# nmndeep/Robust-Segmentation

Hardware: AMD Instinct MI355X
Metric: SEA attack-iterations/sec (UperNet-CNX-T, 512x512) (higher is better)
Workload: dtype f32 (frozen-weight GEMMs on the 16-bit matrix cores by operand splitting: fp16x2 (22 significant bits per operand, 3 MFMA products) forward, fp16x2 (22 significant bits per operand, 3 MFMA products) input gradient; fp32 storage and accumulate)

## Files before the change

include/sea_hip.h:

```cpp
#ifndef SEA_HIP_H
#define SEA_HIP_H

#include <stddef.h>
#include <stdint.h>

#ifdef __cplusplus
extern "C" {
#endif

#define SEA_MODE_MASK_CE 0
#define SEA_MODE_MASK_CE_BAL 1
#define SEA_MODE_JS 2
#define SEA_MODE_CE 3

#define SEA_DTYPE_F32 0
#define SEA_DTYPE_BF16 1
#define SEA_DTYPE_F16 2

#define SEA_LAYOUT_NCHW 0
#define SEA_LAYOUT_NHWC 1

int sea_abi_version(void);
const char* sea_build_info(void);
#define SEA_CONFIG_XCD_ORDER 0
// ... 147 lines not shown
int sea_nhwc_to_nchw(const float* in, const float* scale, const float* residual, float* out, int B, int C,
                     int64_t HW, void* stream);

int sea_patch2x2(const float* src, float* dst, int B, int H, int W, int C, int inverse, void* stream);

int sea_attention_bwd_terms(const float* q, const float* k, const float* v, int64_t sb, int64_t sh, int64_t st, int B, int H,
                            int T, int D, float scale, const float* out, const float* grad_out, const float* lse,
                            float* delta, float* dq, float* dk, float* dv, int64_t gsb, int64_t gsh, int64_t gst,
                            int terms, void* stream);
int sea_attention_fwd_terms(const float* q, const float* k, const float* v, int64_t sb, int64_t sh, int64_t st, int B, int H,
                            int T, int D, float scale, float* out, float* lse, int terms, void* stream);
int sea_attention_fwd_f16(const float* q, const float* k, const float* v, int64_t sb, int64_t sh, int64_t st, int B, int H,
                          int T, int D, float scale, uint32_t* amax_ws, float* out, float* lse, void* stream);
int sea_attention_bwd_f16(const float* q, const float* k, const float* v, int64_t sb, int64_t sh, int64_t st, int B, int H,
                          int T, int D, float scale, const float* out, const float* grad_out, const float* lse,
                          float* delta, uint32_t* amax_ws, float* dq, float* dk, float* dv, int64_t gsb, int64_t gsh,
                          int64_t gst, void* stream);

#define SEA_GEMM_VARIANT_DEFAULT 0u
#define SEA_GEMM_PIPE_SINGLE 1u
#define SEA_GEMM_PIPE_PINGPONG 2u
#define SEA_GEMM_PIPE_BIG 3u
#define SEA_GEMM_PIPE_MASK 3u
#define SEA_GEMM_SHAPE16 4u
int sea_gemm_plan(int M, int N, int K, int terms, int batch, int64_t lda, int64_t ldc, int64_t ld_addend, int prologue, int fused,
                  unsigned variant, int32_t out[16]);
int64_t sea_gemm_split_packed_bytes(int N, int K, int terms);
int sea_absmax_bits(const float* A, int64_t lda, int M, int K, int batch, int64_t strideA, int rows_per_word,
                    uint32_t* out_bits, void* stream);
int sea_gemm_split_f16(const float* A, int64_t lda, const void* Wp, float* C, int64_t ldc, const float* bias, int relu, int M,
                       int N, int K, int batch, int64_t strideA, int64_t strideW_bytes, int64_t strideC,
                       const uint32_t* amax_bits, int amax_rows, uint32_t* out_amax, unsigned variant, void* stream);
int sea_gemm_split_pack(const float* W, int64_t ldw, int trans, int N, int K, int terms, void* out, void* stream);
int sea_gemm_splitk_reduce(const float* partial, int splits, int M, int N, const float* bias, const float* addend,
                           int64_t ld_addend, int relu, float* C, int64_t ldc, uint32_t* out_amax, void* stream);
typedef struct SeaGemmEpilogue {
  const float* addend;
  int64_t ld_addend, stride_addend;
  float* gelu_out;
  const float* gelu_grad_of;
  const float* a_gelu_grad_of;
  int a_gate;
  int a_gelu;
  float a_amax_mul;
  const float* a_amax_mul_dev;
} SeaGemmEpilogue;
int sea_gemm_split_fused(const float* A, int64_t lda, const void* Wp, float* C, int64_t ldc, const float* bias, int relu, int M,
                         int N, int K, int terms, int batch, int64_t strideA, int64_t strideW_bytes, int64_t strideC,
                         const uint32_t* amax_bits, int amax_rows, uint32_t* out_amax, const SeaGemmEpilogue* epi,
                         unsigned variant, void* stream);
int sea_gemm_split(const float* A, int64_t lda, const void* Wp, float* C, int64_t ldc, const float* bias, int relu, int M,
                   int N, int K, int terms, int batch, int64_t strideA, int64_t strideW_bytes, int64_t strideC,
                   unsigned variant, void* stream);
int sea_classifier_supported(int P, int K, int cls);
int sea_classifier_fwd(const float* y, const float* W, const float* bias, float* out, int B, int P, int K, int cls, void* stream);
int sea_classifier_bwd(const float* g, const float* W, float* gy, int B, int P, int K, int cls, const float* gate,
                       const float* gate_scale, void* stream);
int sea_mlp_fused_supported(int C, int H);
int sea_ln_mlp_fused_fwd(const float* x, int64_t ldx, const float* ln_w, const float* ln_b, float ln_eps, const void* W1p,
                         const float* b1, const void* W2p, const float* b2, const float* res, int64_t ldres, float* y,
                         int64_t ldy, int M, int C, int H, const uint32_t* amax_x, const uint32_t* amax_h, void* stream);
int sea_ln_mlp_fused_bwd(const float* g, int64_t ldg, const float* x, int64_t ldx, const float* ln_w, const float* ln_b,
                         float ln_eps, const void* W1p, const float* b1, const void* W2tp, const void* W1tp, float* dx,
                         int64_t lddx, int M, int C, int H, const uint32_t* amax_x, const float* amax_mul_dev, void* stream);
int sea_probe_gelu_mismatches(unsigned long long* out, void* stream);
int sea_probe_ln_rows(const float* x, const float* ln_w, const float* ln_b, float eps, int M, int C, float* yn, float* mean,
                      float* rstd, void* stream);
int sea_mlp_fused_stamps(int bwd, const float* g, int64_t ldg, const float* x, int64_t ldx, const void* W1p, const float* b1,
                         const void* W2p, const void* W1tp, const float* b2, const float* res, float* y, int M, int C,
                         const uint32_t* amax_x, const uint32_t* amax_h, const float* amax_mul_dev, unsigned long long* dbg,
                         void* stream);
int sea_mlp_fused_fwd(const float* x, int64_t ldx, const void* W1p, const float* b1, const void* W2p, const float* b2,
                      const float* res, int64_t ldres, float* y, int64_t ldy, int M, int C, int H, const uint32_t* amax_x,
                      const uint32_t* amax_h, void* stream);
int sea_mlp_fused_bwd(const float* g, int64_t ldg, const float* x, int64_t ldx, const void* W1p, const float* b1,
                      const void* W2tp, const void* W1tp, float* dx, int64_t lddx, int M, int C, int H,
                      const uint32_t* amax_x, const float* amax_mul_dev, void* stream);
int sea_probe_stream_copy(const void* src, void* dst, size_t bytes, int non_temporal, void* stream);
int sea_probe_stream_read(const void* src, float* sink, size_t bytes, void* stream);

#define SEA_MSF_MAX_CLASSES 192
int sea_msf_resize_input(const float* x, float* y, float* y_flip, int64_t planes, int h, int w, int H, int W,
                         void* stream);
int sea_msf_accumulate(const float* logits, float* score, int B, int C, int hl, int wl, int Hs, int Ws, int H, int W,
                       int flip, void* stream);

#define SEA_SW_MAX_ANCHORS 32
int sea_sw_merge(const float* logits, float* out, int B, int C, int hl, int wl, int ws, const int* h_anchors, int n_h,
                 const int* w_anchors, int n_w, int H, int W, int flip, int softmax, int accumulate, void* stream);
int sea_sw_finish(const float* avg, float* score, int B, int C, int H, int W, int Ho, int Wo, int flip, int accumulate,
                  void* stream);

int sea_sw_cut(const float* x, float* crops, int B, int Cx, int ws, const int* h_anchors, int n_h, const int* w_anchors,
               int n_w, int H, int W, void* stream);
int sea_sw_cut_bwd(const float* dcrops, float* dx, int B, int Cx, int ws, const int* h_anchors, int n_h,
                   const int* w_anchors, int n_w, int H, int W, void* stream);
int sea_sw_merge_bwd(const float* g, float* dlogits, int B, int C, int hl, int wl, int ws, const int* h_anchors, int n_h,
                     const int* w_anchors, int n_w, int H, int W, void* stream);

int sea_psp_polyphase_split(const float* x, float* y, int B, int H, int W, int C, int d, int first_only, void* stream);
int sea_psp_polyphase_merge(const float* y, float* x, int B, int H, int W, int C, int d, int first_only, void* stream);
int sea_psp_upsample_ac(const float* x, float* y, int64_t planes, int h, int w, int H, int W, void* stream);
int sea_psp_upsample_ac_bwd(const float* gy, float* gx, float* work, int64_t planes, int h, int w, int H, int W,
                            void* stream);
int sea_psp_upsample_ac_nhwc(const float* x, float* y, int B, int C, int h, int w, int H, int W, int S, void* stream);
int sea_psp_upsample_ac_nhwc_bwd(const float* gy, float* gx, float* work, int B, int C, int h, int w, int H, int W,
// ... 56 lines not shown
```

robust-segmentation_amd/build_native.py:

```python
#!/usr/bin/env python3
from __future__ import annotations

import hashlib
import os
import shutil
import subprocess
import sys
from concurrent.futures import ThreadPoolExecutor

HERE = os.path.dirname(os.path.abspath(__file__))
CSRC = os.path.join(HERE, "csrc")
LIBDIR = os.path.join(HERE, "lib")
OBJDIR = os.path.join(HERE, "build")
LIB = os.path.join(LIBDIR, "libsea_hip.so")
ARCH = "gfx950"

SOURCES = [
    ("linf_kernels.hip", ["-ffp-contract=off"]),
    ("l2_kernels.hip", ["-ffp-contract=off"]),
    ("apgd_control.hip", ["-ffp-contract=off"]),
    ("loss_kernels.hip", []),
    ("loss_stream.hip", []),
    ("loss_split.hip", []),
    ("loss_upsampled.hip", []),
    ("stats_kernels.hip", []),
    ("dwconv_kernels.hip", []),
    ("upsample_kernels.hip", []),
    ("transpose_kernels.hip", ["-ffp-contract=off"]),
    ("wino_kernels.hip", []),
    ("ln_kernels.hip", []),
    ("block_tail.hip", ["-ffp-contract=off"]),
    ("stem_kernels.hip", []),
    ("fpn_fused.hip", []),
    ("probe_kernels.hip", []),
    ("attention.hip", []),
    ("attention_bf16.hip", []),
    ("gemm_split.hip", []),
    ("gemm_split_big.hip", ["-fno-slp-vectorize"]),
    ("gemm_split_pp.hip", ["-fno-slp-vectorize"]),
    ("mlp_fused.hip", ["-fno-slp-vectorize"]),
    ("classifier.hip", []),
    ("msf_kernels.hip", ["-ffp-contract=off"]),
    ("msf_grad.hip", ["-ffp-contract=off"]),
    ("sw_kernels.hip", ["-ffp-contract=off"]),
    ("psp_kernels.hip", []),
    ("bn_train.hip", []),
    ("train_loss.hip", []),
    ("train_loss_up.hip", []),
    ("train_loss_up_pow2.hip", []),
    ("greedy_host.cpp", ["-ffp-contract=off"]),
    ("api_misc.cpp", []),
]
HEADERS = ["sea_common.h", "attention_common.h", "colsum.h", "loss_common.h", "loss_plan.h", "gemm_plan.h", "upsample_plan.h", "launch_grid.h", "gemm_split.h", "bilinear_map.h", "msf_map.h", "train_loss_common.h", os.path.join("..", "..", "include", "sea_hip.h")]


def _hipcc() -> str:
    for cand in (os.environ.get("HIPCC"), shutil.which("hipcc"), "/opt/rocm/bin/hipcc"):
        if cand and os.path.exists(cand):
            return cand
    raise RuntimeError("hipcc not found (set HIPCC)")


def _digest() -> str:
    h = hashlib.sha256()
    for name, flags in SOURCES:
        h.update(open(os.path.join(CSRC, name), "rb").read())
        h.update(" ".join(flags).encode())
    for name in HEADERS:
        h.update(open(os.path.join(CSRC, name), "rb").read())
    return h.hexdigest()[:16]


def build(force: bool = False, verbose: bool = True) -> str:
    stamp_file = os.path.join(LIBDIR, "libsea_hip.stamp")
    digest = _digest()
    if not force and os.path.exists(LIB) and os.path.exists(stamp_file) and open(stamp_file).read() == digest:
        return LIB
    os.makedirs(LIBDIR, exist_ok=True)
    os.makedirs(OBJDIR, exist_ok=True)
    hipcc = _hipcc()
    common = ["-O3", "-fPIC", "-std=c++17", f"--offload-arch={ARCH}", "-Wno-unused-result"]

    hdr = hashlib.sha256()
    for name in HEADERS:
        hdr.update(open(os.path.join(CSRC, name), "rb").read())

    def compile_one(item):
        name, flags = item
        if name == "api_misc.cpp":
            flags = flags + [f'-DSEA_BUILD_STAMP="{digest}"']
        obj = os.path.join(OBJDIR, os.path.splitext(name)[0] + ".o")
        h = hdr.copy()
        h.update(open(os.path.join(CSRC, name), "rb").read())
        h.update(" ".join(common + flags).encode())
        key, keyfile = h.hexdigest(), obj + ".key"
        if not force and os.path.exists(obj) and os.path.exists(keyfile) and open(keyfile).read() == key:
            return obj
        cmd = [hipcc, *common, *flags, "-c", os.path.join(CSRC, name), "-o", obj]
        if verbose:
            print("[build]", " ".join(cmd), flush=True)
        subprocess.run(cmd, check=True)
        with open(keyfile, "w") as f:
            f.write(key)
        return obj

    with ThreadPoolExecutor(max_workers=min(4, len(SOURCES))) as ex:
# ... 15 lines not shown
```

robust-segmentation_amd/semseg/_native.py:

```python
from __future__ import annotations

import ctypes as C
import os
from typing import Optional

import torch

_PKG = os.path.dirname(os.path.dirname(os.path.abspath(__file__)))
LIB_PATH = os.environ.get("SEA_HIP_LIB", os.path.join(_PKG, "lib", "libsea_hip.so"))

MODE_BY_NAME = {"mask-ce-avg": 0, "mask-ce-bal": 1, "js-avg": 2, "ce": 3, "ce-avg": 3}
DTYPE_CODE = {torch.float32: 0, torch.bfloat16: 1, torch.float16: 2}
LAYOUT_NCHW, LAYOUT_NHWC = 0, 1

_lib = None

_vp, _i, _i64, _f, _sz, _u = C.c_void_p, C.c_int, C.c_int64, C.c_float, C.c_size_t, C.c_uint
_SIGS = {
    "sea_abi_version": (C.c_int, []),
    "sea_build_info": (C.c_char_p, []),
    "sea_fastdiv_magic": (_i, [C.c_uint32, C.POINTER(C.c_uint32), C.POINTER(C.c_uint32)]),
    "sea_apgd_linf_step": (_i, [_vp, _vp, _vp, _vp, _vp, _f, _f, _vp, _i, _i64, _vp]),
    "sea_apgd_l2_workspace_bytes": (_i64, [_i]),
    "sea_apgd_l2_step": (_i, [_vp, _vp, _vp, _vp, _vp, _f, _f, _vp, _vp, _i, _i64, _vp]),
# ... 17 lines not shown
    "sea_apgd_track_graph": (_i, [_vp, _vp, _vp, _vp, _i, _i64, _vp, _vp, _vp, _i, _vp, _vp, _vp, _vp, _vp, _vp, _vp, _vp,
                                  _vp, _vp, _vp]),
    "sea_select_copy": (_i, [_vp, _vp, _vp, _vp, _vp, _vp, _vp, _vp, _i, _i, _i64, _i64, _vp]),
    "sea_count_ignored": (_i, [_vp, _i, _i, _i64, _vp, _vp]),
    "sea_worst_miou_greedy": (_i, [_vp, _vp, _i, _i, _i, _vp, _i, _vp, _vp, _vp]),
    "sea_dwconv7x7": (_i, [_vp, _vp, _vp, _vp, _i, _i, _i, _i, _i, _vp]),
    "sea_dwconv7x7_nhwc": (_i, [_vp, _vp, _vp, _vp, _i, _i, _i, _i, _i, _u, _vp]),
    "sea_dwconv7x7_nhwc_add": (_i, [_vp, _vp, _vp, _vp, _vp, _i, _i, _i, _i, _i, _u, _vp]),
    "sea_nchw_to_nhwc": (_i, [_vp, _vp, _vp, _i, _i, _i64, _vp]),
    "sea_nhwc_to_nchw": (_i, [_vp, _vp, _vp, _vp, _i, _i, _i64, _vp]),
    "sea_upsample_bilinear_fwd": (_i, [_vp, _vp, _i64, _i, _i, _i, _i, _vp]),
    "sea_upsample_bilinear_bwd": (_i, [_vp, _vp, _i64, _i, _i, _i, _i, _vp]),
    "sea_layernorm_fwd": (_i, [_vp, _vp, _vp, _vp, _vp, _vp, _i64, _i, _f, _vp]),
    "sea_layernorm_bwd": (_i, [_vp, _vp, _vp, _vp, _vp, _vp, _i64, _i, _vp]),
    "sea_layernorm_bwd_params_workspace": (_i64, [_i64, _i]),
    "sea_layernorm_bwd_params": (_i, [_vp, _vp, _vp, _vp, _vp, _vp, _vp, _vp, _vp, _i64, _i, _vp]),
    "sea_block_tail_fwd": (_i, [_vp, _vp, _vp, _vp, _vp, _i64, _i, _i, _vp]),
    "sea_block_tail_bwd_workspace": (_i64, [_i64, _i]),
    "sea_block_tail_bwd": (_i, [_vp, _vp, _vp, _vp, _vp, _vp, _vp, _i64, _i, _i, _vp]),
    "sea_dwconv7x7_nhwc_wgrad_workspace": (_i64, [_i, _i, _i]),
    "sea_dwconv7x7_nhwc_wgrad": (_i, [_vp, _vp, _vp, _vp, _vp, _i, _i, _i, _i, _vp]),
    "sea_adaptive_avg_pool_nhwc_fwd": (_i, [_vp, _vp, _i, _i, _i, _i, _i, _i, _vp]),
    "sea_adaptive_avg_pool_nhwc_bwd": (_i, [_vp, _vp, _i, _i, _i, _i, _i, _i, _vp]),
    "sea_stem_conv1_ln_gelu": (_i, [_vp, _vp, _vp, _vp, _vp, _vp, _vp, _i, _i, _i, _i, _f, _vp]),
    "sea_stem_conv1_bwd": (_i, [_vp, _vp, _vp, _i, _i, _i, _i, _vp]),
    "sea_ln_gelu_cl_fwd": (_i, [_vp, _vp, _vp, _vp, _i, _i, _i, _i64, _f, _vp]),
    "sea_ln_gelu_cl_bwd": (_i, [_vp, _i, _vp, _vp, _vp, _vp, _i, _i, _i64, _f, _vp]),
    "sea_wino_tiles": (_i64, [_i, _i, _i, _i]),
    "sea_wino_input_transform": (_i, [_vp, _i64, _vp, _vp, _vp, _i64, _i, _i, _i, _i, _i, _i, _vp]),
    "sea_wino_filter_transform": (_i, [_vp, _vp, _i, _i, _i, _i, _vp]),
    "sea_wino_output_transform": (_i, [_vp, _vp, _vp, _vp, _i, _vp, _i, _i, _i, _i, _i, _i, _vp]),
    "sea_tap_gather_fwd": (_i, [_vp, _vp, _i, _i, _i, _i, _i, _i, _i, _i, _vp]),
    "sea_tap_gather_bwd": (_i, [_vp, _vp, _i, _i, _i, _i, _i, _i, _vp]),
    "sea_gate_scale": (_i, [_vp, _vp, _vp, _vp, _i64, _i, _vp]),
    "sea_upsample_bilinear_nhwc_fwd": (_i, [_vp, _vp, _vp, _i, _i, _i, _i, _i, _i, _i64, _vp]),
    "sea_upsample_bilinear_nhwc_bwd": (_i, [_vp, _vp, _i, _i, _i, _i, _i, _i, _i64, _vp]),
    "sea_upsample_plan": (_i, [_i, _i64, _i, _i, _i, _i, _i, _i64, _sz, _sz, _i, _i, C.POINTER(C.c_int32)]),
    "sea_patch2x2": (_i, [_vp, _vp, _i, _i, _i, _i, _i, _vp]),
    "sea_attention_bwd_terms": (_i, [_vp, _vp, _vp, _i64, _i64, _i64, _i, _i, _i, _i, _f, _vp, _vp, _vp, _vp, _vp, _vp, _vp,
                                     _i64, _i64, _i64, _i, _vp]),
    "sea_attention_fwd_terms": (_i, [_vp, _vp, _vp, _i64, _i64, _i64, _i, _i, _i, _i, _f, _vp, _vp, _i, _vp]),
    "sea_attention_fwd_f16": (_i, [_vp, _vp, _vp, _i64, _i64, _i64, _i, _i, _i, _i, _f, _vp, _vp, _vp, _vp]),
    "sea_attention_bwd_f16": (_i, [_vp, _vp, _vp, _i64, _i64, _i64, _i, _i, _i, _i, _f, _vp, _vp, _vp, _vp, _vp, _vp, _vp, _vp,
                                   _i64, _i64, _i64, _vp]),
    "sea_absmax_bits": (_i, [_vp, _i64, _i, _i, _i, _i64, _i, _vp, _vp]),
    "sea_gemm_split_f16": (_i, [_vp, _i64, _vp, _vp, _i64, _vp, _i, _i, _i, _i, _i, _i64, _i64, _i64, _vp, _i, _vp, _u, _vp]),
    "sea_wino_input_transform_amax": (_i, [_vp, _i64, _vp, _vp, _vp, _i64, _i, _i, _i, _i, _i, _i, _vp, _vp]),
    "sea_gemm_split_fused": (_i, [_vp, _i64, _vp, _vp, _i64, _vp, _i, _i, _i, _i, _i, _i, _i64, _i64, _i64, _vp, _i, _vp, _vp, _u, _vp]),
    "sea_gemm_splitk_reduce": (_i, [_vp, _i, _i, _i, _vp, _vp, _i64, _i, _vp, _i64, _vp, _vp]),
    "sea_gemm_split_packed_bytes": (_i64, [_i, _i, _i]),
    "sea_gemm_split_pack": (_i, [_vp, _i64, _i, _i, _i, _i, _vp, _vp]),
    "sea_gemm_split": (_i, [_vp, _i64, _vp, _vp, _i64, _vp, _i, _i, _i, _i, _i, _i, _i64, _i64, _i64, _u, _vp]),
    "sea_gemm_plan": (_i, [_i, _i, _i, _i, _i, _i64, _i64, _i64, _i, _i, _u, C.POINTER(C.c_int32)]),
    "sea_mlp_fused_supported": (_i, [_i, _i]),
    "sea_classifier_supported": (_i, [_i, _i, _i]),
    "sea_classifier_fwd": (_i, [_vp, _vp, _vp, _vp, _i, _i, _i, _i, _vp]),
    "sea_classifier_bwd": (_i, [_vp, _vp, _vp, _i, _i, _i, _i, _vp, _vp, _vp]),
    "sea_probe_gelu_mismatches": (_i, [_vp, _vp]),
    "sea_probe_ln_rows": (_i, [_vp, _vp, _vp, _f, _i, _i, _vp, _vp, _vp, _vp]),
    "sea_mlp_fused_stamps": (_i, [_i, _vp, _i64, _vp, _i64, _vp, _vp, _vp, _vp, _vp, _vp, _vp, _i, _i, _vp, _vp, _vp, _vp, _vp]),
    "sea_mlp_fused_fwd": (_i, [_vp, _i64, _vp, _vp, _vp, _vp, _vp, _i64, _vp, _i64, _i, _i, _i, _vp, _vp, _vp]),
    "sea_mlp_fused_bwd": (_i, [_vp, _i64, _vp, _i64, _vp, _vp, _vp, _vp, _vp, _i64, _i, _i, _i, _vp, _vp, _vp]),
    "sea_ln_mlp_fused_fwd": (_i, [_vp, _i64, _vp, _vp, _f, _vp, _vp, _vp, _vp, _vp, _i64, _vp, _i64, _i, _i, _i, _vp, _vp, _vp]),
    "sea_ln_mlp_fused_bwd": (_i, [_vp, _i64, _vp, _i64, _vp, _vp, _f, _vp, _vp, _vp, _vp, _vp, _i64, _i, _i, _i, _vp, _vp, _vp]),
    "sea_process_config": (_i, [_i]),
    "sea_probe_stream_copy": (_i, [_vp, _vp, _sz, _i, _vp]),
    "sea_probe_stream_read": (_i, [_vp, _vp, _sz, _vp]),
    "sea_msf_resize_input": (_i, [_vp, _vp, _vp, _i64, _i, _i, _i, _i, _vp]),
    "sea_msf_accumulate": (_i, [_vp, _vp, _i, _i, _i, _i, _i, _i, _i, _i, _i, _vp]),
    "sea_psp_polyphase_split": (_i, [_vp, _vp, _i, _i, _i, _i, _i, _i, _vp]),
    "sea_psp_polyphase_merge": (_i, [_vp, _vp, _i, _i, _i, _i, _i, _i, _vp]),
    "sea_psp_upsample_ac": (_i, [_vp, _vp, _i64, _i, _i, _i, _i, _vp]),
    "sea_psp_upsample_ac_bwd": (_i, [_vp, _vp, _vp, _i64, _i, _i, _i, _i, _vp]),
    "sea_psp_upsample_ac_nhwc": (_i, [_vp, _vp, _i, _i, _i, _i, _i, _i, _i, _vp]),
    "sea_psp_upsample_ac_nhwc_bwd": (_i, [_vp, _vp, _vp, _i, _i, _i, _i, _i, _i, _i, _vp]),
    "sea_psp_add_relu": (_i, [_vp, _vp, _vp, _i64, _vp]),
    "sea_psp_add_relu_bwd": (_i, [_vp, _vp, _vp, _i64, _vp]),
    "sea_bn_train_workspace_floats": (_i64, [_i64, _i]),
    "sea_bn_train_fwd": (_i, [_vp, _vp, _vp, _vp, _vp, _vp, _vp, _vp, _vp, _vp, _vp, _vp, _i64, _i, _f, _f, _i, _vp]),
    "sea_bn_train_bwd": (_i, [_vp, _vp, _vp, _vp, _vp, _vp, _vp, _vp, _vp, _vp, _vp, _i64, _i, _i, _vp]),
    "sea_train_ce_workspace_bytes": (_sz, [_i, _i64]),
    "sea_train_ce_fwd": (_i, [_vp, _i, _vp, _vp, _i64, _f, _i, _i, _i, _i64, _vp, _vp, _sz, _vp, _vp]),
    "sea_train_ohem_select": (_i, [_vp, _i64, _vp, _sz, _vp, _vp]),
    "sea_train_ce_bwd": (_i, [_vp, _i, _vp, _vp, _i64, _i, _i, _i, _i64, _vp, _vp, _vp, _vp, _vp]),
    "sea_train_ce_up_tile": (_i, [_i, _i, _i, _i, _i]),
    "sea_train_ce_up_workspace_bytes": (_sz, [_i, _i, _i, _i, _i, _i]),
    "sea_train_ce_up_fwd": (_i, [_vp, _vp, _vp, _i64, _f, _i, _i, _i, _i, _i, _i, _i, _vp, _vp, _sz, _vp, _vp]),
    "sea_train_ce_up_bwd": (_i, [_vp, _vp, _vp, _i64, _i, _i, _i, _i, _i, _i, _i, _vp, _vp, _vp, _vp, _vp, _sz, _vp]),
    "sea_train_ce_up_ac_tile": (_i, [_i, _i, _i, _i, _i]),
    "sea_train_ce_up_ac_workspace_bytes": (_sz, [_i, _i, _i, _i, _i, _i]),
    "sea_train_ce_up_ac_fwd": (_i, [_vp, _vp, _vp, _i64, _f, _i, _i, _i, _i, _i, _i, _i, _vp, _vp, _sz, _vp, _vp]),
    "sea_train_ce_up_ac_bwd": (_i, [_vp, _vp, _vp, _i64, _i, _i, _i, _i, _i, _i, _i, _vp, _vp, _vp, _vp, _vp, _sz, _vp]),
    "sea_train_ce_up_pow2_supported": (_i, [_i, _i, _i, _i, _i]),
    "sea_train_ce_up_pow2_workspace_bytes": (_sz, [_i, _i, _i, _i, _i, _i]),
    "sea_train_ce_up_pow2_fwd": (_i, [_vp, _vp, _vp, _i64, _i, _i, _i, _i, _i, _i, _vp, _vp, _sz, _vp, _vp]),
    "sea_train_ce_up_pow2_scale": (_i, [_vp, _vp, _vp, _vp, _i64, _vp]),
    "sea_sw_merge": (_i, [_vp, _vp, _i, _i, _i, _i, _i, C.POINTER(C.c_int), _i, C.POINTER(C.c_int), _i, _i, _i, _i, _i, _i,
                          _vp]),
    "sea_sw_finish": (_i, [_vp, _vp, _i, _i, _i, _i, _i, _i, _i, _i, _vp]),
    "sea_sw_cut": (_i, [_vp, _vp, _i, _i, _i, C.POINTER(C.c_int), _i, C.POINTER(C.c_int), _i, _i, _i, _vp]),
    "sea_sw_cut_bwd": (_i, [_vp, _vp, _i, _i, _i, C.POINTER(C.c_int), _i, C.POINTER(C.c_int), _i, _i, _i, _vp]),
    "sea_sw_merge_bwd": (_i, [_vp, _vp, _i, _i, _i, _i, _i, C.POINTER(C.c_int), _i, C.POINTER(C.c_int), _i, _i, _i, _vp]),
    "sea_msf_resize_bwd": (_i, [_vp, _vp, _vp, _i64, _i, _i, _i, _i, _i, _vp]),
    "sea_msf_accumulate_bwd": (_i, [_vp, _vp, _vp, _vp, _i, _i, _i, _i, _i, _i, _i, _i, _i, _vp]),
}
EXPORTS = tuple(_SIGS)
# ... 1596 lines not shown
def ksplit_workspace_pin(device):
    return _ksplit_ws.get(device.index if device.index is not None else torch.cuda.current_device())


class _GemmEpilogue(C.Structure):
    _fields_ = [("addend", C.c_void_p), ("ld_addend", C.c_int64), ("stride_addend", C.c_int64),
                ("gelu_out", C.c_void_p), ("gelu_grad_of", C.c_void_p), ("a_gelu_grad_of", C.c_void_p), ("a_gate", C.c_int), ("a_gelu", C.c_int),
                ("a_amax_mul", C.c_float), ("a_amax_mul_dev", C.c_void_p)]


def _amax_words(A3, M, K, G, sA, groups, per_row=False):
    if per_row and G != 1:
        raise SeaNativeError("gemm_split: row_amax (one scale word per row) is defined for a single matrix, not a batch of them")
    if per_row:
        words = torch.empty(M, dtype=torch.int32, device=A3.device)
        _check(lib().sea_absmax_bits(_p(A3), A3.stride(1), M, K, 1, 0, 1, _p(words), _stream()), "sea_absmax_bits")
        return words, 1
    rpw = M // groups if (groups > 1 and M % groups == 0) else 0
    words = torch.empty(groups if rpw else 1, dtype=torch.int32, device=A3.device)
    _check(lib().sea_absmax_bits(_p(A3), A3.stride(1), M, K, G, sA, rpw, _p(words), _stream()), "sea_absmax_bits")
    return words, rpw


_e = os.environ.get("SEA_GEMM_PIPE", "")
GEMM_PIPE = int(_e[0]) if _e[:1] in ("0", "1", "2", "3") else 2
GEMM_MFMA_SHAPE = 16 if os.environ.get("SEA_GEMM_SHAPE", "")[:1] == "1" else 32
del _e
_GEMM_PIPE_BITS = {2: 0, 0: 1, 1: 2, 3: 3}
_GEMM_SHAPE16 = 4


def gemm_variant(pipe=None, mfma_shape=None) -> int:
    pipe = GEMM_PIPE if pipe is None else int(pipe)
    mfma_shape = GEMM_MFMA_SHAPE if mfma_shape is None else int(mfma_shape)
    if pipe not in _GEMM_PIPE_BITS or mfma_shape not in (16, 32):
        raise SeaNativeError("gemm_split: pipe must be 0, 1, 2 or 3 and mfma_shape 16 or 32")
    return _GEMM_PIPE_BITS[pipe] | (_GEMM_SHAPE16 if mfma_shape == 16 else 0)


GEMM_KERNELS = ("single", "pp", "big256", "big384")
_GEMM_PLAN_FIELDS = ("kernel", "terms_t", "f16", "s16", "epi", "pro", "depth", "bm", "bn", "npad", "mblocks", "nblocks", "tiles",
                     "grid", "threads", "lds")


def gemm_plan(M: int, N: int, K: int, terms: int, batch: int = 1, lda=None, ldc=None, ld_add: int = 0, prologue: int = 0,
              fused: bool = False, pipe=None, mfma_shape=None) -> dict:
    out = (C.c_int32 * len(_GEMM_PLAN_FIELDS))()
    rc = lib().sea_gemm_plan(M, N, K, terms, batch, K if lda is None else lda, N if ldc is None else ldc, ld_add, prologue,
                             int(bool(fused)), gemm_variant(pipe, mfma_shape), out)
    plan = dict(zip(_GEMM_PLAN_FIELDS, out), rc=rc)
    return dict(plan, kernel=GEMM_KERNELS[plan["kernel"]], **{k: bool(plan[k]) for k in ("f16", "s16", "epi")})


def gemm_split(A, Wp: PackedWeight, bias=None, relu: bool = False, out=None, amax=None, out_amax=None, addend=None,
               gelu_out=None, gelu_grad_of=None, amax_rows: int = 0, groups: int = 1, a_gelu_grad_of=None,
               a_gelu: bool = False, a_relu_gate=None, row_amax: bool = False, amax_mul: float = 1.0, pipe=None,
               mfma_shape=None):
    variant = gemm_variant(pipe, mfma_shape)
    gate = a_relu_gate is not None
    if gate:
        if a_gelu_grad_of is not None:
            raise SeaNativeError("gemm_split: a_relu_gate and a_gelu_grad_of are exclusive")
        a_gelu_grad_of = a_relu_gate
    _dev(A, bias, out, addend, gelu_out, gelu_grad_of, a_gelu_grad_of)
    batched = Wp.batch > 1 or A.dim() == 3
    A3 = A if A.dim() == 3 else A.unsqueeze(0)
    if (A.dtype != torch.float32 or A3.dim() != 3 or A3.shape[0] != Wp.batch or A3.shape[2] != Wp.K
            or A3.stride(2) != 1):
        raise SeaNativeError("gemm_split: A must be float32 (M,K) / (G,M,K) with K matching the packed weights")
    G, M, K = A3.shape
    if out is None:
        out = torch.empty((G, M, Wp.N) if batched else (M, Wp.N), dtype=torch.float32, device=A.device)
    O3 = out if out.dim() == 3 else out.unsqueeze(0)
    if O3.shape != (G, M, Wp.N) or O3.stride(2) != 1 or out.dtype != torch.float32:
        raise SeaNativeError("gemm_split: output must be float32 (.., M, N) with a contiguous last dim")
    if bias is not None and (bias.dtype != torch.float32 or bias.numel() != Wp.N or not bias.is_contiguous()):
        raise SeaNativeError("gemm_split: bias must be contiguous float32 of N entries")
    sA, sC = (A3.stride(0) if G > 1 else 0), (O3.stride(0) if G > 1 else 0)
    if amax is not None and (amax.dtype != torch.int32 or not amax.is_contiguous()
                             or amax.numel() < (-(-M // amax_rows) if amax_rows > 0 else 1)):
        raise SeaNativeError("gemm_split: amax must hold one int32 word per amax_rows rows")
    mul_dev = amax_mul if (torch.is_tensor(amax_mul) and Wp.terms == 22) else None
    if mul_dev is not None and (mul_dev.dtype != torch.float32 or mul_dev.numel() != 1 or mul_dev.device != A.device):
        raise SeaNativeError("gemm_split: a tensor amax_mul must be one float32 on A's device")
    amax_mul = float(amax_mul) if (Wp.terms == 22 and mul_dev is None) else 1.0
    fused = (addend is not None or gelu_out is not None or gelu_grad_of is not None or a_gelu_grad_of is not None
             or a_gelu or amax_mul != 1.0 or mul_dev is not None)
    if a_gelu_grad_of is not None and (a_gelu_grad_of.shape != A.shape or a_gelu_grad_of.stride() != A.stride()
                                       or a_gelu_grad_of.dtype != torch.float32 or Wp.terms not in (1, 2, 22)):
        raise SeaNativeError("gemm_split: a_gelu_grad_of must be float32 with A's shape and strides (terms 1, 2 or 22)")
    only_pro = gelu_out is None and gelu_grad_of is None
    add_ok = addend is None or (addend.dim() == 2 and addend.shape == O3.shape[1:] and addend.stride(1) == 1
                                and addend.stride(0) % 4 == 0 and addend.data_ptr() % 16 == 0 and addend.dtype == torch.float32)
    if G == 1 and (not fused or (only_pro and add_ok)) and Wp.src is not None and O3.stride(1) % 4 == 0 and O3.data_ptr() % 16 == 0:
        S = _ksplit(M, Wp.N, K)
        if S > 1:
            if Wp.terms == 22 and amax is None:
                amax, amax_rows = _amax_words(A3, M, K, 1, 0, groups, row_amax)
            part = _ksplit_workspace(A.device, S * M * Wp.N).view(S, M, Wp.N)
            shape, strides = (S, M, K // S), (K // S, A3.stride(1), 1)
            gemm_split(A3[0].as_strided(shape, strides), Wp.k_slices(S), out=part, amax=amax, amax_rows=amax_rows,
                       a_gelu_grad_of=None if (a_gelu_grad_of is None or gate) else a_gelu_grad_of.as_strided(shape, strides),
                       a_gelu=a_gelu, amax_mul=mul_dev if mul_dev is not None else amax_mul, pipe=pipe, mfma_shape=mfma_shape,
                       **({"a_relu_gate": a_gelu_grad_of.as_strided(shape, strides)} if gate else {}))
            _check(lib().sea_gemm_splitk_reduce(_p(part), S, M, Wp.N, _p(bias), _p(addend),
                                                addend.stride(0) if addend is not None else 0, int(relu), _p(O3), O3.stride(1),
                                                _p(out_amax) if Wp.terms == 22 else None, _stream()), "sea_gemm_splitk_reduce")
            return out
    if addend is not None and (a_gelu or a_gelu_grad_of is not None):
        out = gemm_split(A, Wp, bias=bias, relu=False, out=out, amax=amax, out_amax=None, amax_rows=amax_rows, groups=groups,
                         a_gelu_grad_of=None if gate else a_gelu_grad_of, a_gelu=a_gelu,
                         a_relu_gate=a_gelu_grad_of if gate else None, row_amax=row_amax,
                         amax_mul=mul_dev if mul_dev is not None else amax_mul, pipe=pipe, mfma_shape=mfma_shape)
        out += addend
        if relu:
            torch.relu_(out)
        if out_amax is not None and Wp.terms == 22:
            O2 = out if out.dim() == 3 else out.unsqueeze(0)
            _check(lib().sea_absmax_bits(_p(O2), O2.stride(1), M, Wp.N, G, sC, 0, _p(out_amax), _stream()), "sea_absmax_bits")
        return out
    if fused:
        epi = _GemmEpilogue()
        if addend is not None:
            D3 = addend if addend.dim() == 3 else addend.unsqueeze(0)
            if D3.shape != O3.shape or D3.stride(2) != 1 or addend.dtype != torch.float32:
                raise SeaNativeError("gemm_split: addend must be float32 of the output's shape with a contiguous last dim")
            epi.addend, epi.ld_addend, epi.stride_addend = D3.data_ptr(), D3.stride(1), (D3.stride(0) if G > 1 else 0)
        for name, t in (("gelu_out", gelu_out), ("gelu_grad_of", gelu_grad_of)):
            if t is not None:
                T3 = t if t.dim() == 3 else t.unsqueeze(0)
                if T3.shape != O3.shape or T3.stride() != O3.stride() or t.dtype != torch.float32:
                    raise SeaNativeError(f"gemm_split: {name} must be float32 with the output's shape and strides")
                setattr(epi, name, T3.data_ptr())
        if a_gelu_grad_of is not None:
            epi.a_gelu_grad_of = a_gelu_grad_of.data_ptr()
            epi.a_gate = int(gate)
        epi.a_gelu = int(bool(a_gelu))
        epi.a_amax_mul = amax_mul if amax_mul != 1.0 else 0.0
        epi.a_amax_mul_dev = mul_dev.data_ptr() if mul_dev is not None else None
        if Wp.terms == 22 and amax is None:
            amax, amax_rows = _amax_words(A3, M, K, G, sA, groups, row_amax)
        _check(lib().sea_gemm_split_fused(_p(A3), A3.stride(1), _p(Wp.data), _p(O3), O3.stride(1), _p(bias), int(relu), M, Wp.N,
                                          K, Wp.terms, G, sA, Wp.stride, sC, _p(amax) if Wp.terms == 22 else None, amax_rows,
                                          _p(out_amax) if Wp.terms == 22 else None, C.addressof(epi), variant, _stream()),
               "sea_gemm_split_fused")
        return out
    if Wp.terms == 22:
        if amax is None:
            amax, amax_rows = _amax_words(A3, M, K, G, sA, groups, row_amax)
        _check(lib().sea_gemm_split_f16(_p(A3), A3.stride(1), _p(Wp.data), _p(O3), O3.stride(1), _p(bias), int(relu), M, Wp.N,
                                        K, G, sA, Wp.stride, sC, _p(amax), amax_rows, _p(out_amax), variant, _stream()),
# ... 6 lines not shown
```

Measured before the change: 571.1.

## Add row-panel GEMM kernel that reduces K-splits in LDS instead of separate pass

Adds a new kernel for N=384 split-K GEMMs with terms 22. Each block owns a 32-row panel, waves split K into 2 or 4 slices, and partial sums are combined in shared memory before the bias, addend, relu and amax epilogue. This replaces the separate split-K partial GEMM plus reduce launch and removes the workspace round trip through global memory. It is enabled by default through SEA_GEMM_ROWS. The trade-off is fewer blocks (M/32) and a large LDS footprint, which may limit occupancy.

New measurement: 566.5. Within noise of the previous version (-0.8%).

```diff
diff --git a/devtools/gemm_rows_ab.py b/devtools/gemm_rows_ab.py
--- /dev/null
+++ b/devtools/gemm_rows_ab.py
@@ -0,0 +1,41 @@
+import os
+import sys
+
+import torch
+
+sys.path.insert(0, os.path.join(os.path.dirname(os.path.abspath(__file__)), "..", "robust-segmentation_amd"))
+from semseg import _native as N
+
+M, K, NN = 8192, 1536, 384
+g = torch.Generator(device="cuda").manual_seed(3)
+W = torch.randn(NN, K, generator=g, device="cuda") / K ** 0.5
+Wp = N.gemm_split_pack(W, terms=22)
+bias = torch.randn(NN, generator=g, device="cuda")
+A = torch.randn(M, K, generator=g, device="cuda") * (torch.rand(M, 1, generator=g, device="cuda") * 4 + 0.01)
+t = torch.randn(M, K, generator=g, device="cuda") * 2
+add = torch.randn(M, NN, generator=g, device="cuda")
+rowbits = A.abs().amax(1).contiguous().view(torch.int32)
+imgbits = A.abs().view(8, -1).amax(1).contiguous().view(torch.int32)
+mul = torch.full((1,), 1.13, device="cuda")
+cases = {
+    "plain": dict(amax=imgbits, amax_rows=1024, bias=bias),
+    "a_gelu+addend": dict(a_gelu=True, addend=add, bias=bias, amax=imgbits, amax_rows=1024),
+    "a_gelu_grad_of": dict(a_gelu_grad_of=t, amax=rowbits, amax_rows=1, amax_mul=mul),
+}
+print("lib", N.LIB_PATH, flush=True)
+for name, kw in cases.items():
+    res = {}
+    for rows in (False, True):
+        out = torch.empty(M, NN, device="cuda")
+        for _ in range(20):
+            N.gemm_split(A, Wp, out=out, rows=rows, **kw)
+        torch.cuda.synchronize()
+        e0, e1 = torch.cuda.Event(enable_timing=True), torch.cuda.Event(enable_timing=True)
+        e0.record()
+        for _ in range(300):
+            N.gemm_split(A, Wp, out=out, rows=rows, **kw)
+        e1.record()
+        torch.cuda.synchronize()
+        res[rows] = (e0.elapsed_time(e1) / 300 * 1e3, out)
+    print(f"{name:16s} slices+reduce {res[False][0]:7.1f} us   rows {res[True][0]:7.1f} us   equal {torch.equal(res[False][1], res[True][1])}",
+          flush=True)
diff --git a/include/sea_hip.h b/include/sea_hip.h
--- a/include/sea_hip.h
+++ b/include/sea_hip.h
@@ -223,6 +223,12 @@
 int sea_gemm_split(const float* A, int64_t lda, const void* Wp, float* C, int64_t ldc, const float* bias, int relu, int M,
                    int N, int K, int terms, int batch, int64_t strideA, int64_t strideW_bytes, int64_t strideC,
                    unsigned variant, void* stream);
+int sea_gemm_rows_plan(int M, int N, int K, int splits, int terms, int prologue, int fused_out, int64_t lda, int64_t ldc,
+                       int64_t ld_addend, size_t a_addr, size_t c_addr, size_t addend_addr, size_t bias_addr, int32_t out[4]);
+int sea_gemm_split_rows(const float* A, int64_t lda, const void* Wp, float* C, int64_t ldc, const float* bias, int relu, int M,
+                        int N, int K, int terms, int batch, int64_t strideA, int64_t strideW_bytes, int64_t strideC,
+                        const uint32_t* amax_bits, int amax_rows, uint32_t* out_amax, const SeaGemmEpilogue* epi,
+                        unsigned variant, int splits, void* stream);
 int sea_classifier_supported(int P, int K, int cls);
 int sea_classifier_fwd(const float* y, const float* W, const float* bias, float* out, int B, int P, int K, int cls, void* stream);
 int sea_classifier_bwd(const float* g, const float* W, float* gy, int B, int P, int K, int cls, const float* gate,
diff --git a/robust-segmentation_amd/build_native.py b/robust-segmentation_amd/build_native.py
--- a/robust-segmentation_amd/build_native.py
+++ b/robust-segmentation_amd/build_native.py
@@ -38,6 +38,7 @@
     ("gemm_split.hip", []),
     ("gemm_split_big.hip", ["-fno-slp-vectorize"]),
     ("gemm_split_pp.hip", ["-fno-slp-vectorize"]),
+    ("gemm_split_rows.hip", ["-fno-slp-vectorize"]),
     ("mlp_fused.hip", ["-fno-slp-vectorize"]),
     ("classifier.hip", []),
     ("msf_kernels.hip", ["-ffp-contract=off"]),
@@ -51,7 +52,7 @@
     ("greedy_host.cpp", ["-ffp-contract=off"]),
     ("api_misc.cpp", []),
 ]
-HEADERS = ["sea_common.h", "attention_common.h", "colsum.h", "loss_common.h", "loss_plan.h", "gemm_plan.h", "upsample_plan.h", "launch_grid.h", "gemm_split.h", "bilinear_map.h", "msf_map.h", "train_loss_common.h", os.path.join("..", "..", "include", "sea_hip.h")]
+HEADERS = ["sea_common.h", "attention_common.h", "colsum.h", "loss_common.h", "loss_plan.h", "gemm_plan.h", "gemm_rows_plan.h", "upsample_plan.h", "launch_grid.h", "gemm_split.h", "bilinear_map.h", "msf_map.h", "train_loss_common.h", os.path.join("..", "..", "include", "sea_hip.h")]
 
 
 def _hipcc() -> str:
diff --git a/robust-segmentation_amd/csrc/gemm_rows_plan.h b/robust-segmentation_amd/csrc/gemm_rows_plan.h
--- /dev/null
+++ b/robust-segmentation_amd/csrc/gemm_rows_plan.h
@@ -0,0 +1,55 @@
+#pragma once
+#include <stddef.h>
+#include <stdint.h>
+
+#ifndef SEA_ERR_ARG
+#define SEA_ERR_ARG 1
+#endif
+
+namespace sea {
+
+constexpr int kRowsPanel = 32;
+constexpr int kRowsWaves = 8;
+constexpr int kRowsMinKb = 8;
+constexpr int kRowsMaxM = 8448;
+
+struct GemmRowsQuery {
+  int M, N, K, splits, terms ;
+  int pro;
+  bool fused_out;
+  int64_t lda, ldc, ld_add;
+  size_t a_addr, c_addr, add_addr, bias_addr;
+};
+struct GemmRowsPlan {
+  int applies;
+  int nt, nsplit;
+  int grid, threads;
+  size_t lds;
+};
+
+static inline int gemm_rows_plan(const GemmRowsQuery& q, GemmRowsPlan* p) {
+  *p = GemmRowsPlan{};
+  if (q.M <= 0 || q.N <= 0 || q.K <= 0 || q.splits < 1 || (q.K % (32 * q.splits)) != 0) return SEA_ERR_ARG;
+  if (q.lda < q.K || q.ldc < q.N || q.pro < 0 || q.pro > 3 || (q.ld_add != 0 && q.ld_add < q.N)) return SEA_ERR_ARG;
+  const int S = q.splits;
+  bool ok = q.N == 384;
+  ok = ok && (S == 2 || S == 4);
+  ok = ok && (q.K / (32 * S)) >= kRowsMinKb;
+  ok = ok && q.terms == 22;
+  ok = ok && q.pro <= 2 && !q.fused_out;
+  ok = ok && q.M <= kRowsMaxM;
+  ok = ok && (q.lda % 4) == 0 && (q.ldc % 4) == 0 && (q.ld_add % 4) == 0;
+  ok = ok && ((q.a_addr | q.c_addr | q.add_addr | q.bias_addr) & 15) == 0;
+  ok = ok && (q.add_addr == 0) == (q.ld_add == 0);
+  ok = ok && q.lda <= ((1ll << 30) - 1) / q.M && q.ldc <= ((1ll << 30) - 1) / q.M && q.ld_add <= ((1ll << 30) - 1) / q.M;
+  if (!ok) return 0;
+  p->applies = 1;
+  p->nt = q.N / 32;
+  p->nsplit = kRowsWaves / S;
+  p->grid = (q.M + kRowsPanel - 1) / kRowsPanel;
+  p->threads = 64 * kRowsWaves;
+  p->lds = (size_t)2 * S * 2 * kRowsPanel * 64 + (size_t)kRowsPanel * q.N * 4 + 2 * kRowsPanel * 4;
+  return 0;
+}
+
+}
diff --git a/robust-segmentation_amd/csrc/gemm_split_rows.hip b/robust-segmentation_amd/csrc/gemm_split_rows.hip
--- /dev/null
+++ b/robust-segmentation_amd/csrc/gemm_split_rows.hip
@@ -0,0 +1,338 @@
+#include "gemm_split.h"
+#include "gemm_rows_plan.h"
+
+namespace sea {
+
+template <int S, int NT32, int PRO>
+__global__ __launch_bounds__(64 * kRowsWaves) void gemm_split_rows_kernel(const GemmSplitArgs p) {
+  constexpr int NTHR = 64 * kRowsWaves;
+  constexpr int NSPLIT = kRowsWaves / S, TN = NT32 / NSPLIT;
+  constexpr int N = 32 * NT32, N4 = N / 4;
+  constexpr int IMG = kRowsPanel * 64;
+  constexpr int STAGE = S * 2 * IMG;
+  constexpr int NA = S * (kRowsPanel * 8) / NTHR;
+  constexpr int SSTEP = S / NA;
+  constexpr int SLOTS = 3 * TN;
+  constexpr int UNIT_EVERY = SLOTS / (3 * NA);
+  constexpr bool HAS_T = PRO == 1;
+  constexpr int DA = HAS_T ? 1 : 2;
+  static_assert(S * NSPLIT == kRowsWaves && TN * NSPLIT == NT32 && NA >= 1 && NA * SSTEP == S && SLOTS % (3 * NA) == 0, "configuration");
+  static_assert((kRowsPanel * N4) % NTHR == 0, "combine: whole trips");
+  extern __shared__ __attribute__((aligned(16))) char smem[];
+  float* const part = (float*)(smem + 2 * STAGE);
+  float* const row_sc = part + kRowsPanel * N;
+  float* const row_inv = row_sc + kRowsPanel;
+
+  const int M = p.M, Npad = p.Npad;
+  const int64_t lda = p.lda;
+  const int Ks = p.K / S, nkb = Ks / GS_BK;
+  const int m0 = (int)blockIdx.x * kRowsPanel;
+  const int tid = threadIdx.x, lane = tid & 63;
+  const int wave_u = __builtin_amdgcn_readfirstlane(tid >> 6);
+  const int ws = wave_u / NSPLIT, wc = wave_u % NSPLIT;
+  const int r = lane & 31, h = lane >> 5;
+  const int q = tid & 7, arow = (tid >> 3) & 31, sl0 = tid >> 8;
+
+  const int row_g = (m0 + arow < M) ? m0 + arow : M - 1;
+  const float* const Arow = p.A + (int64_t)row_g * lda + sl0 * Ks + 4 * q;
+  const float* const Trow = HAS_T ? p.a_gelu_grad_of + (int64_t)row_g * lda + sl0 * Ks + 4 * q : nullptr;
+  const uint32_t a_wr0 = (uint32_t)(sl0 * 2 * IMG + arow * 64 + swz<false>(arow, q >> 1) + (q & 1) * 8);
+  const uint32_t a_rd = (uint32_t)(ws * 2 * IMG + r * 64 + swz<false>(r, h));
+
+  const int64_t w_term = (int64_t)Npad * 64, w_kb = 2 * w_term;
+  const char* const Wbase = p.W + (int64_t)ws * p.strideW + (int64_t)(wc * TN * 32) * 64;
+  const uint32_t w_bytes = (uint32_t)((int64_t)nkb * w_kb - (int64_t)(wc * TN * 32) * 64);
+  const __amdgpu_buffer_rsrc_t w_rs = __builtin_amdgcn_make_buffer_rsrc((void*)Wbase, 0, (int)w_bytes, 0x00020000);
+  const uint32_t w_voff = (uint32_t)(r * 64 + h * 16);
+
+  struct Raw {
+    f32x4 a[NA];
+    f32x4 t[HAS_T ? NA : 1];
+  };
+  Raw R0 = {}, R1 = {};
+  auto fetch_a = [&](Raw& R, int kb) __attribute__((always_inline)) {
+    const int kbc = kb < nkb ? kb : nkb - 1;
+#pragma unroll
+    for (int i = 0; i < NA; ++i) R.a[i] = *(const f32x4*)(Arow + i * SSTEP * Ks + kbc * GS_BK);
+    if constexpr (HAS_T) {
+#pragma unroll
+      for (int i = 0; i < NA; ++i) R.t[i] = *(const f32x4*)(Trow + i * SSTEP * Ks + kbc * GS_BK);
+    }
+  };
+  bf16x8 fa[2][2], fb[TN][2][2];
+  auto fetch_b = [&](int kb, int ni) __attribute__((always_inline)) {
+    const int kbc = kb < nkb ? kb : nkb - 1;
+#pragma unroll
+    for (int t = 0; t < 2; ++t)
+#pragma unroll
+      for (int s = 0; s < 2; ++s)
+        fb[ni][s][t] = __builtin_bit_cast(bf16x8, __builtin_amdgcn_raw_buffer_load_b128(
+                                                      w_rs, (int)w_voff, kbc * (int)w_kb + t * (int)w_term + ni * 2048 + s * 32, 0));
+  };
+  auto read_a = [&](const char* stage) __attribute__((always_inline)) {
+#pragma unroll
+    for (int s = 0; s < 2; ++s)
+#pragma unroll
+      for (int t = 0; t < 2; ++t) fa[s][t] = *(const bf16x8*)(stage + ((a_rd ^ (uint32_t)(32 * s)) + t * IMG));
+  };
+
+  float a_sc = 1.f;
+  f32x4 sv;
+  uint32_t hi_a, hi_b;
+  auto unit_a = [&](Raw& R, int i, int part_, char* stage) __attribute__((always_inline)) {
+    if (part_ == 0) {
+      f32x4 v = R.a[i];
+      if constexpr (PRO == 1) {
+#pragma unroll
+        for (int e = 0; e < 4; ++e) v[e] *= gelu_grad_f(R.t[i][e]);
+      }
+      if constexpr (PRO == 2) {
+#pragma unroll
+        for (int e = 0; e < 4; ++e) v[e] = gelu_f(v[e]);
+      }
+#pragma unroll
+      for (int e = 0; e < 4; ++e) v[e] *= a_sc;
+      hi_a = pack_f16(v[0], v[1]);
+      hi_b = pack_f16(v[2], v[3]);
+      sv = v;
+    } else if (part_ == 1) {
+      const f32x2 f0 = __builtin_convertvector(__builtin_bit_cast(f16x2, hi_a), f32x2);
+      const f32x2 f1 = __builtin_convertvector(__builtin_bit_cast(f16x2, hi_b), f32x2);
+      sv[0] -= f0[0];
+      sv[1] -= f0[1];
+      sv[2] -= f1[0];
+      sv[3] -= f1[1];
+    } else {
+      *(u32x2*)(stage + a_wr0 + i * SSTEP * 2 * IMG) = u32x2{hi_a, hi_b};
+      *(u32x2*)(stage + IMG + a_wr0 + i * SSTEP * 2 * IMG) = u32x2{pack_f16(sv[0], sv[1]), pack_f16(sv[2], sv[3])};
+    }
+  };
+  f32x16 acc[TN];
+#pragma unroll
+  for (int ni = 0; ni < TN; ++ni)
+#pragma unroll
+    for (int e = 0; e < 16; ++e) acc[ni][e] = 0.f;
+  auto mfma3 = [&](int s, int ni, int j) __attribute__((always_inline)) {
+    const int ia = j == 0 ? 1 : 0, ib = j == 1 ? 1 : 0;
+    acc[ni] = __builtin_amdgcn_mfma_f32_32x32x16_f16(__builtin_bit_cast(f16x8, fa[s][ia]), __builtin_bit_cast(f16x8, fb[ni][s][ib]),
+                                                     acc[ni], 0, 0, 0);
+  };
+
+#define SEA_PIN() __builtin_amdgcn_sched_barrier(0)
+  auto step = [&](char* nxt, Raw& Rn, int kb, int kf) __attribute__((always_inline)) {
+    int unit = 0;
+    SEA_PIN();
+#pragma unroll
+    for (int ni = 0; ni < TN; ++ni) {
+#pragma unroll
+      for (int s = 0; s < 2; ++s) {
+#pragma unroll
+        for (int j = 0; j < 3; ++j) {
+          mfma3(s, ni, j);
+          const int slot = (ni * 2 + s) * 3 + j;
+          if (slot % UNIT_EVERY == 0 && unit < 3 * NA) {
+            unit_a(Rn, unit / 3, unit % 3, nxt);
+            ++unit;
+          } else if (unit == 3 * NA) {
+            fetch_a(Rn, kf);
+            ++unit;
+          }
+          SEA_PIN();
+        }
+      }
+      fetch_b(kb + 1, ni);
+      SEA_PIN();
+    }
+    __syncthreads();
+    read_a(nxt);
+    SEA_PIN();
+  };
+
+  Raw& RA = R0;
+  Raw& RB = DA == 2 ? R1 : R0;
+  fetch_a(R0, 0);
+  if constexpr (DA == 2) fetch_a(R1, 1);
+#pragma unroll
+  for (int ni = 0; ni < TN; ++ni) fetch_b(0, ni);
+  if (tid < kRowsPanel) {
+    int row = m0 + tid;
+    row = row < M ? row : M - 1;
+    float sc, inv;
+    uint32_t word = p.amax_bits[p.amax_rows > 0 ? row / p.amax_rows : 0];
+    const float mul = p.amax_mul_dev ? *p.amax_mul_dev : p.amax_mul;
+    if (mul != 1.f) word = __float_as_uint(__uint_as_float(word) * mul) & 0x7fffffffu;
+    pow2_scale(word, sc, inv);
+    row_sc[tid] = sc;
+    row_inv[tid] = inv;
+  }
+  __syncthreads();
+  a_sc = row_sc[arow];
+  char* const st0 = smem;
+  char* const st1 = smem + STAGE;
+#pragma unroll
+  for (int i = 0; i < NA; ++i) {
+    unit_a(R0, i, 0, st0);
+    unit_a(R0, i, 1, st0);
+    unit_a(R0, i, 2, st0);
+  }
+  fetch_a(R0, DA);
+  __syncthreads();
+  read_a(st0);
+  int kb = 0;
+  for (; kb + 2 <= nkb; kb += 2) {
+    step(st1, RB, kb, kb + 1 + DA);
+    step(st0, RA, kb + 1, kb + 2 + DA);
+  }
+  if (kb < nkb) step(st1, RB, kb, nkb);
+#undef SEA_PIN
+
+  {
+    const float* const w_inv = (const float*)(p.W + (int64_t)ws * p.strideW + (int64_t)nkb * w_kb);
+    f32x4 ri[4];
+#pragma unroll
+    for (int j = 0; j < 4; ++j) ri[j] = *(const f32x4*)(row_inv + 8 * j + 4 * h);
+#pragma unroll
+    for (int ni = 0; ni < TN; ++ni) {
+      const float wi = w_inv[wc * TN * 32 + ni * 32 + r];
+#pragma unroll
+      for (int e = 0; e < 16; ++e)
+        acc[ni][e] = acc[ni][e] * (ri[e >> 2][e & 3] * wi) + 0.f;
+    }
+  }
+  {
+    float* const mine = part + wc * TN * 32 + r;
+#pragma unroll
+    for (int s = 0; s < S; ++s) {
+      if (ws == s) {
+#pragma unroll
+        for (int ni = 0; ni < TN; ++ni)
+#pragma unroll
+          for (int e = 0; e < 16; ++e) {
+            float* const at = mine + ((e & 3) + 8 * (e >> 2) + 4 * h) * N + ni * 32;
+            *at = s == 0 ? acc[ni][e] : *at + acc[ni][e];
+          }
+      }
+      __syncthreads();
+    }
+  }
+
+  const f32x4* const part4 = (const f32x4*)part;
+  const f32x4* const bias4 = (const f32x4*)p.bias;
+  const int relu = p.relu;
+  uint32_t omax = 0;
+#pragma unroll
+  for (int k = 0; k < kRowsPanel * N4 / NTHR; ++k) {
+    const int f = k * NTHR + tid;
+    const int row_l = f / N4, c4 = f - row_l * N4;
+    const int row = m0 + row_l;
+    f32x4 v = part4[f];
+    if (row >= M) continue;
+    if (bias4) v += bias4[c4];
+    if (p.addend) v += *(const f32x4*)(p.addend + (int64_t)row * p.ld_add + 4 * c4);
+    if (relu) {
+#pragma unroll
+      for (int e = 0; e < 4; ++e) v[e] = v[e] > 0.f ? v[e] : 0.f;
+    }
+    *(f32x4*)(p.C + (int64_t)row * p.ldc + 4 * c4) = v;
+#pragma unroll
+    for (int e = 0; e < 4; ++e) {
+      const uint32_t vb = __float_as_uint(v[e]) & 0x7fffffffu;
+      omax = vb > omax ? vb : omax;
+    }
+  }
+  if (p.out_amax != nullptr) {
+#pragma unroll
+    for (int o = 32; o > 0; o >>= 1) {
+      const uint32_t other = (uint32_t)__shfl_xor((int)omax, o, 64);
+      omax = other > omax ? other : omax;
+    }
+    if (lane == 0 && omax > *(volatile uint32_t*)p.out_amax) atomicMax(p.out_amax, omax);
+  }
+}
+
+template <auto KERN>
+static inline void rows_launch(const GemmSplitArgs& p, const GemmRowsPlan& pl, hipStream_t st) {
+  static bool attr_set_dev[64] = {};
+  int dev = 0;
+  (void)hipGetDevice(&dev);
+  if (!attr_set_dev[dev & 63]) {
+    (void)hipFuncSetAttribute((const void*)KERN, hipFuncAttributeMaxDynamicSharedMemorySize, (int)pl.lds);
+    attr_set_dev[dev & 63] = true;
+  }
+  hipLaunchKernelGGL(KERN, dim3(pl.grid), dim3(pl.threads), pl.lds, st, p);
+}
+
+}
+
+using namespace sea;
+
+extern "C" int sea_gemm_rows_plan(int M, int N, int K, int splits, int terms, int prologue, int fused_out, int64_t lda, int64_t ldc,
+                                  int64_t ld_addend, size_t a_addr, size_t c_addr, size_t addend_addr, size_t bias_addr,
+                                  int32_t out[4]) {
+  SEA_CHECK_ARG(out != nullptr);
+  GemmRowsPlan pl;
+  const int rc = gemm_rows_plan(GemmRowsQuery{M, N, K, splits, terms, prologue, fused_out != 0, lda, ldc, ld_addend, a_addr, c_addr,
+                                              addend_addr, bias_addr}, &pl);
+  out[0] = pl.applies;
+  out[1] = pl.grid;
+  out[2] = pl.threads;
+  out[3] = (int32_t)pl.lds;
+  return rc;
+}
+
+extern "C" int sea_gemm_split_rows(const float* A, int64_t lda, const void* Wp, float* C, int64_t ldc, const float* bias, int relu,
+                                   int M, int N, int K, int terms, int batch, int64_t strideA, int64_t strideW_bytes, int64_t strideC,
+                                   const uint32_t* amax_bits, int amax_rows, uint32_t* out_amax, const SeaGemmEpilogue* epi,
+                                   unsigned variant, int splits, void* stream) {
+  (void)strideA;
+  (void)strideC;
+  SEA_CHECK_ARG(A && Wp && C && amax_bits && amax_rows >= 0 && batch == 1 && variant == 0u);
+  SEA_CHECK_ARG((((uintptr_t)Wp) & 15) == 0 && (strideW_bytes % 16) == 0);
+  const float* const a_t = epi ? epi->a_gelu_grad_of : nullptr;
+  const bool a_gelu = epi && epi->a_gelu;
+  SEA_CHECK_ARG(!(a_gelu && a_t) && (((uintptr_t)a_t) & 15) == 0);
+  const int pro = a_gelu ? 2 : (a_t ? (epi->a_gate ? 3 : 1) : 0);
+  const float* const addend = epi ? epi->addend : nullptr;
+  GemmRowsPlan pl;
+  SEA_CHECK_ARG(gemm_rows_plan(GemmRowsQuery{M, N, K, splits, terms, pro, epi && (epi->gelu_out || epi->gelu_grad_of), lda, ldc,
+                                             addend ? epi->ld_addend : 0, (size_t)(uintptr_t)A, (size_t)(uintptr_t)C,
+                                             (size_t)(uintptr_t)addend, (size_t)(uintptr_t)bias}, &pl) == 0 && pl.applies);
+  const int npad = (N + GS_BN - 1) / GS_BN * GS_BN;
+  SEA_CHECK_ARG(strideW_bytes >= (int64_t)(K / splits / GS_BK) * 2 * npad * GS_BK * 2 + (int64_t)npad * 8);
+  GemmSplitArgs p = {};
+  p.A = A;
+  p.W = (const char*)Wp;
+  p.C = C;
+  p.bias = bias;
+  p.lda = lda;
+  p.ldc = ldc;
+  p.strideW = strideW_bytes;
+  p.M = M;
+  p.N = N;
+  p.K = K;
+  p.Npad = npad;
+  p.relu = relu;
+  p.amax_bits = amax_bits;
+  p.amax_rows = amax_rows;
+  p.amax_mul = 1.f;
+  p.out_amax = out_amax;
+  if (epi) {
+    p.addend = addend;
+    p.ld_add = epi->ld_addend;
+    p.a_gelu_grad_of = a_t;
+    p.a_gelu = epi->a_gelu;
+    if (epi->a_amax_mul > 0.f) p.amax_mul = epi->a_amax_mul;
+    p.amax_mul_dev = epi->a_amax_mul_dev;
+  }
+  const hipStream_t st = (hipStream_t)stream;
+  constexpr auto key = [](int s, int nt, int pro_) { return s | nt << 3 | pro_ << 8; };
+#define SEA_ROWS_CASE(S_, NT_, PRO_) \
+  case key(S_, NT_, PRO_): rows_launch<gemm_split_rows_kernel<S_, NT_, PRO_>>(p, pl, st); break;
+  switch (key(splits, pl.nt, pro)) {
+    SEA_ROWS_CASE(4, 12, 0) SEA_ROWS_CASE(4, 12, 1) SEA_ROWS_CASE(4, 12, 2)
+    SEA_ROWS_CASE(2, 12, 0) SEA_ROWS_CASE(2, 12, 1) SEA_ROWS_CASE(2, 12, 2)
+    default: return SEA_ERR_ARG;
+  }
+#undef SEA_ROWS_CASE
+  SEA_RETURN_LAST();
+}
diff --git a/robust-segmentation_amd/semseg/_native.py b/robust-segmentation_amd/semseg/_native.py
--- a/robust-segmentation_amd/semseg/_native.py
+++ b/robust-segmentation_amd/semseg/_native.py
@@ -93,6 +93,9 @@
     "sea_gemm_split_pack": (_i, [_vp, _i64, _i, _i, _i, _i, _vp, _vp]),
     "sea_gemm_split": (_i, [_vp, _i64, _vp, _vp, _i64, _vp, _i, _i, _i, _i, _i, _i, _i64, _i64, _i64, _u, _vp]),
     "sea_gemm_plan": (_i, [_i, _i, _i, _i, _i, _i64, _i64, _i64, _i, _i, _u, C.POINTER(C.c_int32)]),
+    "sea_gemm_rows_plan": (_i, [_i, _i, _i, _i, _i, _i, _i, _i64, _i64, _i64, _sz, _sz, _sz, _sz, C.POINTER(C.c_int32)]),
+    "sea_gemm_split_rows": (_i, [_vp, _i64, _vp, _vp, _i64, _vp, _i, _i, _i, _i, _i, _i, _i64, _i64, _i64, _vp, _i, _vp, _vp, _u, _i,
+                                 _vp]),
     "sea_mlp_fused_supported": (_i, [_i, _i]),
     "sea_classifier_supported": (_i, [_i, _i, _i]),
     "sea_classifier_fwd": (_i, [_vp, _vp, _vp, _vp, _i, _i, _i, _i, _vp]),
@@ -1795,10 +1798,42 @@
     return dict(plan, kernel=GEMM_KERNELS[plan["kernel"]], **{k: bool(plan[k]) for k in ("f16", "s16", "epi")})
 
 
+GEMM_ROWS = os.environ.get("SEA_GEMM_ROWS", "1") != "0"
+
+
+def gemm_rows_plan(M: int, N: int, K: int, splits: int, terms: int = 22, prologue: int = 0, fused_out: bool = False, lda=None,
+                   ldc=None, ld_add: int = 0, a_addr: int = 0, c_addr: int = 0, add_addr: int = 0, bias_addr: int = 0) -> dict:
+    out = (C.c_int32 * 4)()
+    rc = lib().sea_gemm_rows_plan(M, N, K, splits, terms, prologue, int(bool(fused_out)), K if lda is None else lda,
+                                  N if ldc is None else ldc, ld_add, a_addr, c_addr, add_addr, bias_addr, out)
+    return dict(rc=rc, applies=bool(out[0]), grid=out[1], threads=out[2], lds=out[3])
+
+
+def gemm_split_rows(A, Wp: PackedWeight, splits: int, out, amax, amax_rows: int = 0, bias=None, relu: bool = False, out_amax=None,
+                    addend=None, a_gelu_grad_of=None, a_gelu: bool = False, amax_mul=1.0):
+    _dev(A, out, bias, addend, a_gelu_grad_of, amax)
+    M, K = A.shape
+    epi = _GemmEpilogue()
+    if addend is not None:
+        epi.addend, epi.ld_addend = addend.data_ptr(), addend.stride(0)
+    if a_gelu_grad_of is not None:
+        epi.a_gelu_grad_of = a_gelu_grad_of.data_ptr()
+    epi.a_gelu = int(bool(a_gelu))
+    if torch.is_tensor(amax_mul):
+        epi.a_amax_mul_dev = amax_mul.data_ptr()
+    else:
+        epi.a_amax_mul = float(amax_mul) if float(amax_mul) != 1.0 else 0.0
+    Ws = Wp.k_slices(splits)
+    _check(lib().sea_gemm_split_rows(_p(A), A.stride(0), _p(Ws.data), _p(out), out.stride(0), _p(bias), int(relu), M, Wp.N, K,
+                                     Wp.terms, 1, 0, Ws.stride, 0, _p(amax), amax_rows, _p(out_amax), C.addressof(epi), 0,
+                                     splits, _stream()), "sea_gemm_split_rows")
+    return out
+
+
 def gemm_split(A, Wp: PackedWeight, bias=None, relu: bool = False, out=None, amax=None, out_amax=None, addend=None,
                gelu_out=None, gelu_grad_of=None, amax_rows: int = 0, groups: int = 1, a_gelu_grad_of=None,
                a_gelu: bool = False, a_relu_gate=None, row_amax: bool = False, amax_mul: float = 1.0, pipe=None,
-               mfma_shape=None):
+               mfma_shape=None, rows=None):
     variant = gemm_variant(pipe, mfma_shape)
     gate = a_relu_gate is not None
     if gate:
@@ -1840,6 +1875,15 @@
         if S > 1:
             if Wp.terms == 22 and amax is None:
                 amax, amax_rows = _amax_words(A3, M, K, 1, 0, groups, row_amax)
+            if (GEMM_ROWS if rows is None else bool(rows)) and variant == 0 and not gate and Wp.terms == 22:
+                plan = gemm_rows_plan(M, Wp.N, K, S, Wp.terms, 2 if a_gelu else (1 if a_gelu_grad_of is not None else 0), False,
+                                      A3.stride(1), O3.stride(1), addend.stride(0) if addend is not None else 0, A3.data_ptr(),
+                                      O3.data_ptr(), addend.data_ptr() if addend is not None else 0,
+                                      bias.data_ptr() if bias is not None else 0)
+                if plan["rc"] == 0 and plan["applies"]:
+                    gemm_split_rows(A3[0], Wp, S, O3[0], amax, amax_rows, bias=bias, relu=relu, out_amax=out_amax, addend=addend,
+                                    a_gelu_grad_of=a_gelu_grad_of, a_gelu=a_gelu, amax_mul=mul_dev if mul_dev is not None else amax_mul)
+                    return out
             part = _ksplit_workspace(A.device, S * M * Wp.N).view(S, M, Wp.N)
             shape, strides = (S, M, K // S), (K // S, A3.stride(1), 1)
             gemm_split(A3[0].as_strided(shape, strides), Wp.k_slices(S), out=part, amax=amax, amax_rows=amax_rows,
```
